# anovos/anovos

Measured on AMD Instinct MI355X. Metric: rows/sec (whole node) full analyzer+drift+transform, higher is better.
Workload: dtype fp32 data + fp64 accumulators; 1 GPU; model=anovos-full-pipeline, rows_per_gpu=125000000, n_cols=201, global_batch=125000000, parallelism=dp1

## Files before the change

anovos_amd/data_analyzer/quality_checker.py:

```python

from __future__ import annotations

import re
import warnings
from typing import Dict, List

import numpy as np
import pandas as pd
import torch

from anovos_amd.core import dist
from anovos_amd.core.dtypes import NULL_CODE
from anovos_amd.core.frame import AnovosFrame, Column
from anovos_amd.data_analyzer.stats_generator import (
    measures_of_cardinality,
    missingCount_computation,
    mode_computation,
    uniqueCount_computation,
)
from anovos_amd.data_transformer.transformers import _load_model, _save_model, imputation_MMM
from anovos_amd.ops import histogram as hist_ops
from anovos_amd.ops import rowops
from anovos_amd.ops import stats as stats_ops
from anovos_amd.shared.utils import attributeType_segregation, get_dtype, normalize_columns
# ... 51 lines not shown

@traced
def nullRows_detection(ctx, idf, list_of_cols="all", drop_cols=[], treatment=False, treatment_threshold=0.8, print_impact=False):
    if list_of_cols == "all":
        num_cols, cat_cols, _ = attributeType_segregation(idf)
        list_of_cols = num_cols + cat_cols
    cols = normalize_columns(idf, list_of_cols, drop_cols)
    if len(cols) == 0:
        raise TypeError("Invalid input for Column(s)")
    treatment = _parse_bool(treatment)
    treatment_threshold = float(treatment_threshold)
    if treatment_threshold < 0 or treatment_threshold > 1:
        raise TypeError("Invalid input for Treatment Threshold Value")

    counts = rowops.row_null_counts(idf, cols)
    if treatment_threshold == 1:
        flagged = counts == len(cols)
    else:
        flagged = counts > (len(cols) * treatment_threshold)

    total = idf.count()
    key = counts.to(torch.int32) * 2 + flagged.to(torch.int32)
    size = (len(cols) + 1) * 2
    from anovos_amd.ops import backend as _backend

    if key.is_cuda and _backend.use_hip(key):
        hist = _backend.hip_ext().code_counts(key.contiguous(), size).to(torch.float64)
    else:
        hist = torch.bincount(key.to(torch.long), minlength=size).to(torch.float64)
    dist.all_reduce_(hist, "sum")
    hist_l = hist.cpu().numpy().tolist()
    rows = []
    for nc in range(len(cols) + 1):
        for fl in (0, 1):
            c = hist_l[nc * 2 + fl]
            if c > 0:
                rows.append([nc, int(c), round(c / total, 4), fl])
    odf_print = pd.DataFrame(rows, columns=["null_cols_count", "row_count", "row_pct", "flagged"])

    if treatment:
        odf = idf.filter_rows(~flagged)
        odf_print = odf_print.rename(columns={"flagged": "treated"})
    else:
        odf = idf
    if print_impact:
        print(odf_print.to_string(index=False))
    return odf, odf_print


@traced
def nullColumns_detection(
    ctx,
    idf,
    list_of_cols="missing",
    drop_cols=[],
    treatment=False,
# ... 566 lines not shown
```

anovos_amd/ops/distinct.py:

```python

from __future__ import annotations

import math
from typing import Dict, List

import torch

from anovos_amd.core import dist
from anovos_amd.ops import backend
from anovos_amd.ops.groupby import _mix64

HLL_P = 12
HLL_M = 1 << HLL_P


def hll_registers(t: torch.Tensor, p: int = None) -> torch.Tensor:
    p = HLL_P if p is None else p
    m = 1 << p
    if t.is_cuda and backend.use_hip(t):
        ext = backend.hip_ext()
        return ext.hll_registers(t.contiguous(), p)
    v = t[~torch.isnan(t)]
    if v.dtype == torch.float32:
        x = v.view(torch.int32).to(torch.int64) & 0xFFFFFFFF
# ... 50 lines not shown
    zeros = int((regs == 0).sum())
    if e <= 2.5 * m and zeros:
        e = m * math.log(m / zeros)
    return e


def approx_distinct(idf, cols: List[str]) -> Dict[str, int]:
    out = {}
    if not cols:
        return out
    first = idf.col(cols[0]).data
    if first.is_cuda and backend.use_hip(first):
        ext = backend.hip_ext()
        cold = [c for c in cols if "moments" not in idf.col(c).cache]
        if len(cold) >= max(2, len(cols) // 2):
            from anovos_amd.ops import stats as stats_ops

            tensors = [idf.col(c).data.contiguous() for c in cols]
            shifts = stats_ops.compute_column_shifts(tensors)
            mom_local, flat = ext.moments_hll(tensors, HLL_P, shifts)
            glob = stats_ops.merge_moments_global(mom_local).numpy().tolist()
            for i, c in enumerate(cols):
                idf.col(c).cache.setdefault("moments", stats_ops.MomentStats(glob[i], shift=shifts[i]))
        else:
            flat = ext.hll_registers_multi([idf.col(c).data.contiguous() for c in cols], HLL_P)
    else:
        flat = torch.stack([hll_registers(idf.col(c).data) for c in cols]).to(torch.int32)
    dist.all_reduce_(flat, "max")
    regs = flat.cpu().numpy()
    import numpy as np

    m = float(HLL_M)
    z = np.power(2.0, -regs.astype(np.float64)).sum(axis=1)
    alpha = 0.7213 / (1 + 1.079 / m)
    e = alpha * m * m / z
# ... 31 lines not shown
```

anovos_amd/ops/groupby.py:

```python

from __future__ import annotations

from typing import Dict, List, Optional, Tuple

import torch

from anovos_amd.core import dist
from anovos_amd.core.dtypes import NULL_CODE
from anovos_amd.ops import backend


def align_dictionaries(idf, cols: List[str]) -> None:
    if not dist.is_dist():
        return
    cat = [
        c for c in cols
        if idf.col(c).kind == "categorical" and "dict_aligned" not in idf.col(c).cache
    ]
    if not cat:
        return
    import hashlib

    sigs = []
    for c in cat:
# ... 16 lines not shown
        col.cache.clear()
    for c in cat:
        idf.col(c).cache["dict_aligned"] = True


def cat_value_counts(idf, cols: List[str]) -> Dict[str, torch.Tensor]:
    align_dictionaries(idf, cols)
    out = {}
    cached = [c for c in cols if "cat_counts" in idf.col(c).cache]
    for c in cached:
        out[c] = idf.col(c).cache["cat_counts"]
    cols = [c for c in cols if c not in set(cached)]
    bufs = []
    gpu_cols = [c for c in cols if idf.col(c).data.is_cuda and backend.use_hip(idf.col(c).data)]
    if gpu_cols:
        ext = backend.hip_ext()
        sizes = [len(idf.col(c).dictionary or []) for c in gpu_cols]
        flat_multi = ext.code_counts_multi([idf.col(c).data.contiguous() for c in gpu_cols], sizes)
        gpu_cnt = {}
        off = 0
        for c, size in zip(gpu_cols, sizes):
            gpu_cnt[c] = flat_multi[off : off + size]
            gpu_cnt[c + "\0null"] = flat_multi[off + size : off + size + 1]
            off += size + 1
    for c in cols:
        col = idf.col(c)
        size = len(col.dictionary or [])
        codes = col.data
        if c in gpu_cols:
            cnt = gpu_cnt[c]
        else:
            valid = codes[codes != NULL_CODE].long()
            cnt = torch.bincount(valid, minlength=size) if size else torch.zeros(0, dtype=torch.int64, device=codes.device)
# ... 202 lines not shown
```

anovos_amd/ops/hip/anovos_bindings.hip:

```cpp

#include <torch/extension.h>
#include <c10/hip/HIPStream.h>
#include <hip/hip_runtime.h>

#include <algorithm>
#include <cstdlib>
#include <cstring>
#include <vector>

#include "anovos_kernels.h"

namespace {

hipStream_t current_stream() { return c10::hip::getCurrentHIPStream().stream(); }

void check_hip(int err, const char *what) {
  TORCH_CHECK(err == 0, what, " failed: ", hipGetErrorString((hipError_t)err));
}

int pick_chunks(int64_t n, int ncols) {
  int64_t by_size = (n + (1 << 16) - 1) >> 16;
  int64_t cap = std::max<int64_t>(1, 16384 / std::max(1, ncols));
  int64_t c = std::min<int64_t>(std::max<int64_t>(by_size, 1), cap);
  int64_t floor_c = std::min<int64_t>(by_size, std::max<int64_t>(1, 2048 / std::max(1, ncols)));
// ... 118 lines not shown
};

CutoffTable cutoff_table(const std::vector<torch::Tensor> &cutoffs, const std::vector<int64_t> &idx) {
  CutoffTable ct;
  for (int64_t i : idx) {
    auto cc = cutoffs[i].to(torch::kFloat64).cpu().contiguous();
    const double *cd = cc.data_ptr<double>();
    ct.offs.push_back((int64_t)ct.flat.size());
    ct.flat.insert(ct.flat.end(), cd, cd + cc.numel());
    ct.lens.push_back((int)cc.numel());
    ct.max_ncut = std::max(ct.max_ncut, (int)cc.numel());
  }
  return ct;
}

std::tuple<torch::Tensor, torch::Tensor> moments_body(const std::vector<torch::Tensor> &cols,
                                                      const std::vector<double> &shifts,
                                                      int64_t p, const char *name) {
  ColumnBatch all = gather_columns(cols, name, F32 | F64);
  if (!shifts.empty()) check_count(shifts.size(), cols.size(), name, "shifts");
  auto device = all.device;
  const bool hll = p >= 0;
  const int64_t m = hll ? (int64_t)1 << p : 0;
  auto mom = torch::zeros({all.ncols(), 9}, on(device, torch::kFloat64));
  torch::Tensor regs, reg_sub;
  if (hll) regs = torch::zeros({all.ncols(), m}, on(device, torch::kInt32));
  for (auto &b : split_by_dtype(all)) {
    int ncols = b.ncols();
    int nchunks = pick_chunks(b.maxn, ncols);
    auto dptr = upload(b.ptrs, device);
    auto dlen = upload(b.lens, device);
    auto dsh = upload(shifts.empty() ? std::vector<double>(ncols, 0.0) : pick(shifts, b.idx), device);
    auto partials = torch::empty({(int64_t)ncols * nchunks, 9}, on(device, torch::kFloat64));
    auto sub = torch::empty({ncols, 9}, on(device, torch::kFloat64));
    if (hll) {
      reg_sub = torch::zeros({ncols, m}, on(device, torch::kInt32));
      check_hip(anovos_moments_hll(ptr_table<const void>(dptr), dlen.data_ptr<int64_t>(),
                                   dsh.data_ptr<double>(), ncols, (int)p, nchunks, b.dtype,
                                   partials.data_ptr<double>(), sub.data_ptr<double>(),
                                   reg_sub.data_ptr<int>(), current_stream()),
                "anovos_moments_hll");
    } else {
      check_hip(anovos_moments(ptr_table<const void>(dptr), dlen.data_ptr<int64_t>(),
                               dsh.data_ptr<double>(), ncols, nchunks, b.dtype,
                               partials.data_ptr<double>(), sub.data_ptr<double>(),
                               current_stream()),
                "anovos_moments");
    }
    auto didx = upload(b.idx, device);
    mom.index_copy_(0, didx, sub);
    if (hll) regs.index_copy_(0, didx, reg_sub);
  }
  return {mom, regs};
}

// ... 68 lines not shown
  auto doff = upload(offs, b.device);
  auto dflat = upload(flat, b.device);
  check_hip(launch(ptr_table<const int32_t>(dptr), dlen.data_ptr<int64_t>(), b.ncols(),
                   dflat.template data_ptr<T>(), doff.data_ptr<int64_t>(), nchunks,
                   ptr_table<T>(dout), current_stream()),
            name);
  return outs;
}

}

torch::Tensor column_moments(std::vector<torch::Tensor> cols, std::vector<double> shifts) {
  return std::get<0>(moments_body(cols, shifts, -1, "column_moments"));
}

std::tuple<torch::Tensor, torch::Tensor> moments_hll(std::vector<torch::Tensor> cols, int64_t p,
                                                     std::vector<double> shifts) {
  TORCH_CHECK(p >= 0, "moments_hll: p must not be negative");
  return moments_body(cols, shifts, p, "moments_hll");
}

torch::Tensor column_histograms(std::vector<torch::Tensor> cols, torch::Tensor lo,
                                torch::Tensor hi, int64_t nbins) {
  ColumnBatch all = gather_columns(cols, "column_histograms", F32 | F64);
  auto device = all.device;
  auto lo_d = device_f64(lo, cols.size(), all, "lo");
  auto hi_d = device_f64(hi, cols.size(), all, "hi");
  auto out = torch::zeros({all.ncols(), nbins}, on(device, torch::kInt64));
  for (auto &b : split_by_dtype(all)) {
    int nchunks = pick_chunks(b.maxn, b.ncols());
    auto dptr = upload(b.ptrs, device);
    auto dlen = upload(b.lens, device);
    auto didx = upload(b.idx, device);
    auto sub = torch::zeros({b.ncols(), nbins}, on(device, torch::kInt64));
// ... 70 lines not shown
  check_hip(anovos_code_counts(codes.data_ptr<int32_t>(), codes.numel(), (int)size, nchunks,
                               (uint64_t *)out.data_ptr<int64_t>(), current_stream()),
            "anovos_code_counts");
  return out;
}

torch::Tensor hll_registers(torch::Tensor x, int64_t p) {
  ColumnBatch b = gather_columns({x}, "hll_registers", F32 | F64);
  auto regs = torch::zeros({(int64_t)1 << p}, on(b.device, torch::kInt32));
  if (x.numel() == 0) return regs;
  int nchunks = std::min(pick_chunks(x.numel(), 1), 4096);
  check_hip(anovos_hll(x.data_ptr(), x.numel(), (int)p, nchunks, b.dtype,
                       regs.data_ptr<int32_t>(), current_stream()),
            "anovos_hll");
  return regs;
}

void row_null_counts_num(std::vector<torch::Tensor> cols, torch::Tensor out) {
  ColumnBatch all = gather_columns(cols, "row_null_counts_num", F32 | F64 | I32, true);
  check_dense_on_device(out, all, "out", torch::kInt32, all.maxn);
  for (auto &b : split_by_dtype(all)) {
    auto dptr = upload(b.ptrs, b.device);
    check_hip(anovos_row_null(ptr_table<const void>(dptr), b.ncols(), out.numel(), b.dtype,
                              out.data_ptr<int32_t>(), current_stream()),
              "anovos_row_null");
  }
}

torch::Tensor hll_registers_multi(std::vector<torch::Tensor> cols, int64_t p) {
  ColumnBatch all = gather_columns(cols, "hll_registers_multi", F32 | F64);
// ... 168 lines not shown
              "anovos_centered_gram_sr");
    return gram;
  }
  int row_chunks = (int)std::min<int64_t>(std::max<int64_t>(1, 2048 / std::max(npairs, 1)),
                                          std::max<int64_t>(1, n >> 16));
  row_chunks = std::max(row_chunks, 1);
  auto partials = torch::empty({(int64_t)npairs * row_chunks, 256}, on(device, torch::kFloat32));
  check_hip(anovos_centered_gram(ptr_table<const void>(dptr), n, k, means_d.data_ptr<float>(),
                                 pi.data_ptr<int>(), pj.data_ptr<int>(), npairs, row_chunks,
                                 partials.data_ptr<float>(), gram.data_ptr<float>(),
                                 current_stream()),
            "anovos_centered_gram");
  return gram;
}

torch::Tensor code_counts_multi(std::vector<torch::Tensor> cols, std::vector<int64_t> sizes) {
  ColumnBatch b = gather_columns(cols, "code_counts_multi", I32);
  check_count(sizes.size(), cols.size(), b.name, "sizes");
  std::vector<int64_t> offs;
  int64_t off = 0;
  int lds_slots = 0;
  for (int64_t s : sizes) {
    TORCH_CHECK(s >= 0 && s < INT32_MAX, b.name, ": dictionary size out of range");
    offs.push_back(off);
    off += s + 1;
    if (s + 1 <= CODE_LDS_SLOTS) lds_slots = std::max(lds_slots, (int)s + 1);
  }
  int nchunks = pick_chunks(b.maxn, b.ncols());
  auto out = torch::zeros({off}, on(b.device, torch::kInt64));
  auto dptr = upload(b.ptrs, b.device);
  auto dlen = upload(b.lens, b.device);
  auto doff = upload(offs, b.device);
  auto dsz = upload(std::vector<int>(sizes.begin(), sizes.end()), b.device);
  check_hip(anovos_code_counts_multi(ptr_table<const int32_t>(dptr), dlen.data_ptr<int64_t>(),
                                     doff.data_ptr<int64_t>(), dsz.data_ptr<int>(), b.ncols(),
                                     lds_slots, nchunks, (uint64_t *)out.data_ptr<int64_t>(),
                                     current_stream()),
            "anovos_code_counts_multi");
  return out;
}

namespace {

struct PairPlan {
  std::vector<int64_t> items;
  std::vector<int64_t> offs;
  int64_t total = 0;
  int nitems = 0;
  int lds_slots = 0;
  int64_t col_reads = 0;
};

PairPlan plan_pair_items(const std::vector<int64_t> &sizes, const std::vector<int64_t> &pair_i,
                         const std::vector<int64_t> &pair_j) {
// ... 308 lines not shown
    auto sub = torch::zeros({b.ncols(), 2}, on(device, torch::kInt64));
    torch::Tensor dout;
    if (mode) dout = upload(out_ptrs(outs, b), device);
    check_hip(anovos_outlier_clamp(ptr_table<const void>(dptr), dlen.data_ptr<int64_t>(),
                                   b.ncols(), lo_sel.data_ptr<double>(), hi_sel.data_ptr<double>(),
                                   nchunks, (int)mode, b.dtype,
                                   mode ? ptr_table<void>(dout) : nullptr,
                                   (uint64_t *)sub.data_ptr<int64_t>(), current_stream()),
              "anovos_outlier_clamp");
    counts.index_copy_(0, didx, sub);
  }
  return {counts, outs};
}

PYBIND11_MODULE(TORCH_EXTENSION_NAME, m) {
  m.def("code_counts_multi", &code_counts_multi, "fused multi-column code counts + null slot (K5)");
  m.def("pair_code_counts", &pair_code_counts, "contingency tables of code-column pairs (K22)");
  m.def("pair_code_counts_plan", &pair_code_counts_plan,
        "[items, column streams, LDS counters] of a K22 pair list");
  m.def("grouped_moments", &grouped_moments, "(n, s1, s2) of value columns per code slot (K23)");
  m.def("grouped_moments_plan", &grouped_moments_plan,
        "[items, column streams, accumulator cells] of a K23 pair list");
  m.attr("GRP_CELLS") = GRP_CELLS;
  m.def("outlier_clamp_columns", &outlier_clamp_columns, "fused outlier count/clamp (K10/K11)");
  m.def("label_counts_multi", &label_counts_multi, "fused multi-column label-conditioned histograms (K9)");
  m.def("bucketize_label_counts", &bucketize_label_counts, "fused bucketize + label counts, no binned materialization (K6+K9)");
  m.def("moments_hll", &moments_hll, "fused moments + HLL registers (K1/K2+K4)",
        py::arg("cols"), py::arg("p"), py::arg("shifts") = std::vector<double>());
  m.def("centered_gram_bf16", &centered_gram_bf16, "bf16 MFMA centered Gram X^T X (K8)");
  m.def("bracket_histograms_grouped", &bracket_histograms_grouped, "grouped refinement histograms (K3)");
  m.def("bucketize_columns_float", &bucketize_columns_float, "bucketize to float bin labels (K6)");
  m.def("bucketize_columns_float_counts", &bucketize_columns_float_counts,
        "bucketize to float bin labels + per-column bin counts from the same pass (K6)");
  m.def("lut_apply_f32", &lut_apply_f32, "fused LUT gather -> float (K12)");
  m.def("lut_apply_i32", &lut_apply_i32, "fused LUT gather -> int32 (K12)");
  m.def("hll_registers_multi", &hll_registers_multi, "fused multi-column HLL (K4)");
  m.def("scale_columns", &scale_columns, "fused (x-a)*b scaling (K11)");
  m.def("fill_nan_columns", &fill_nan_columns, "fused NaN fill (K11)");
  m.def("fill_code_columns", &fill_code_columns, "fused categorical null fill (K11)");
  m.def("column_moments", &column_moments, "fused per-column moments (K1/K2)",
        py::arg("cols"), py::arg("shifts") = std::vector<double>());
  m.def("column_histograms", &column_histograms, "fused per-column histograms (K3/K6)");
  m.def("bracket_histograms", &bracket_histograms, "quantile-refinement histograms (K3)");
  m.def("bucketize_columns", &bucketize_columns, "branchless bucketize (K6)");
  m.def("code_counts", &code_counts, "dictionary code bincount (K5)");
  m.def("hll_registers", &hll_registers, "HyperLogLog registers (K4)");
  m.def("row_null_counts_num", &row_null_counts_num, "fused row null counts (K10)");
}
```

anovos_amd/ops/hip/anovos_kernels.h:

```cpp

#pragma once

#include <hip/hip_runtime.h>
#include <cstdint>


constexpr int CODE_LDS_SLOTS = 16384;
constexpr int PAIR_LDS_SLOTS = 16384;
constexpr int PAIR_PMAX = 8;
constexpr int PAIR_ITEM_WORDS = 4 + 4 * PAIR_PMAX;
constexpr int GRP_CELLS = 16;
constexpr int GRP_PMAX = 8;
constexpr int GRP_THREADS = 256;
constexpr int GRP_CELL_BYTES = 20;
constexpr int GRP_ITEM_WORDS = 5 + 2 * GRP_PMAX;
constexpr int RB_BINS = 512;
constexpr int RB_MAXB = 16;
constexpr int LABEL_MAX_SLOTS = 8192;
constexpr int BKT_COUNTS_MAX_NCUT = 4096;


extern "C" {
int anovos_moments(const void *const *cols, const int64_t *lens,
                   const double *shifts, int ncols, int nchunks, int dtype,
                   double *partials, double *out, hipStream_t stream);
int anovos_hist(const void *const *cols, const int64_t *lens, int ncols,
                const double *lo, const double *hi, int nbins, int nchunks,
                int dtype, uint64_t *out, hipStream_t stream);
int anovos_bracket_hist(const void *const *cols, const int64_t *lens,
                        const int64_t *colidx, int nbrackets, const double *lo,
                        const double *hi, int nbins, int nchunks, int dtype,
                        uint64_t *out, hipStream_t stream);
int anovos_bucketize(const void *const *cols, const int64_t *lens, int ncols,
                     const double *cutflat, const int64_t *cutoff_off,
// ... 28 lines not shown
                                  const int *cutoff_len, int max_ncut, int nchunks, int dtype,
                                  float *const *outs, uint64_t *counts, const int64_t *count_off,
                                  hipStream_t stream);
int anovos_lut_apply_f32(const int32_t *const *cols, const int64_t *lens, int ncols,
                         const float *lutflat, const int64_t *lut_off, int nchunks,
                         float *const *outs, hipStream_t stream);
int anovos_lut_apply_i32(const int32_t *const *cols, const int64_t *lens, int ncols,
                         const int32_t *lutflat, const int64_t *lut_off, int nchunks,
                         int32_t *const *outs, hipStream_t stream);
int anovos_fill_code(const int32_t *const *cols, const int64_t *lens, int ncols,
                     const int32_t *fill, int nchunks, int32_t *const *outs,
                     hipStream_t stream);
int anovos_code_counts_multi(const int32_t *const *cols, const int64_t *lens,
                             const int64_t *offs, const int *sizes, int ncols,
                             int lds_slots, int nchunks, uint64_t *out,
                             hipStream_t stream);
int anovos_outlier_clamp(const void *const *cols, const int64_t *lens,
                         int ncols, const double *lo, const double *hi,
                         int nchunks, int mode, int dtype, void *const *outs,
                         uint64_t *counts, hipStream_t stream);
int anovos_moments_hll(const void *const *cols, const int64_t *lens,
                       const double *shifts, int ncols, int p, int nchunks,
                       int dtype, double *partials, double *mom_out,
                       int32_t *regs, hipStream_t stream);
int anovos_bucketize_label_counts(const void *const *cols, const uint8_t *label,
                                  const int64_t *lens, const double *cutflat,
                                  const int64_t *cutoff_off, const int *cutoff_len,
                                  const int64_t *offs, const int *sizes, int ncols,
                                  int max_ncut, int max_slots, int nchunks,
                                  int dtype, uint64_t *out, hipStream_t stream);
int anovos_label_counts_multi(const void *const *cols, const uint8_t *label,
                              const int64_t *lens, const int64_t *offs,
                              const int *sizes, const int *dtypes, int ncols,
                              int max_slots, int nchunks, uint64_t *out,
                              hipStream_t stream);
int anovos_centered_gram(const void *const *cols, int64_t n, int k,
                         const float *means, const int *pair_i,
                         const int *pair_j, int npairs, int row_chunks,
                         float *partials, float *gram, hipStream_t stream);
// ... 14 lines not shown
```

anovos_amd/ops/hip/anovos_kernels.hip:

```cpp

#include <hip/hip_runtime.h>
#include <cfloat>
#include <cstdint>
#include <cmath>

#include "anovos_kernels.h"

#define THREADS 256
#define DEV_INLINE __device__ __forceinline__

typedef int nat_i4 __attribute__((ext_vector_type(4)));
typedef float nat_f4 __attribute__((ext_vector_type(4)));


#define NSTAT 9

struct MomAcc {
  double n, s1, s2, s3, s4, mn, mx, zn, nf;
};

DEV_INLINE void mom_add(MomAcc &a, double v, double shift) {
  if (!isnan(v)) {
    a.n += 1.0;
    double d = v - shift;
    a.s1 += d;
    double d2 = d * d;
    a.s2 += d2;
// ... 750 lines not shown
  __syncthreads();
  for (int c = c0; c < c1; ++c) {
    const T *__restrict__ x = cols[c] + s;
    for (int i = threadIdx.x; i < nr; i += THREADS)
      if (is_null_elem(x[i])) rc[i] += 1;
  }
  __syncthreads();
  if (ncolchunks == 1) {
    for (int i = threadIdx.x; i < nr; i += THREADS) out[s + i] += (int32_t)rc[i];
  } else {
    for (int i = threadIdx.x; i < nr; i += THREADS)
      if (rc[i]) atomicAdd(&out[s + i], (int32_t)rc[i]);
  }
}


template <typename T>
__global__ __launch_bounds__(THREADS) void hll_multi_kernel(
    const T *const *cols, const int64_t *lens, int p, int nchunks,
    int32_t *regs ) {
  extern __shared__ int32_t sreg[];
  const int m = 1 << p;
  const int col = blockIdx.x / nchunks;
  const int chunk = blockIdx.x % nchunks;
  for (int i = threadIdx.x; i < m; i += THREADS) sreg[i] = 0;
  __syncthreads();
  const T *__restrict__ x = cols[col];
  const int64_t n = lens[col];
  const int64_t per = (n + nchunks - 1) / nchunks;
  const int64_t s = (int64_t)chunk * per;
// ... 342 lines not shown
                   void *const *outs, hipStream_t stream) {
  dim3 grid(ncols * nchunks);
  if (dtype == 0)
    hipLaunchKernelGGL(fillnan_kernel<float>, grid, dim3(THREADS), 0, stream,
                       (const float *const *)cols, lens, fill, nchunks,
                       (float *const *)outs);
  else
    hipLaunchKernelGGL(fillnan_kernel<double>, grid, dim3(THREADS), 0, stream,
                       (const double *const *)cols, lens, fill, nchunks,
                       (double *const *)outs);
  return (int)hipGetLastError();
}

}

__global__ __launch_bounds__(THREADS) void code_counts_multi_kernel(
    const int32_t *const *cols, const int64_t *lens, const int64_t *offs,
    const int *sizes, int nchunks, uint64_t *out) {
  const int col = blockIdx.x / nchunks;
  const int chunk = blockIdx.x % nchunks;
  const int32_t *__restrict__ codes = cols[col];
  const int64_t n = lens[col];
  const int size = sizes[col];
  const int slots = size + 1;
  uint64_t *base = out + offs[col];

  extern __shared__ uint32_t cnt[];
  const bool use_lds = (slots <= CODE_LDS_SLOTS);
  if (use_lds) {
    for (int i = threadIdx.x; i < slots; i += THREADS) cnt[i] = 0;
    __syncthreads();
  }
  const int64_t per = (n + nchunks - 1) / nchunks;
  const int64_t s = (int64_t)chunk * per;
  const int64_t e = min(n, s + per);
  if (use_lds) {
    const int64_t nv = (e - s) / 4;
    const nat_i4 *__restrict__ cv = reinterpret_cast<const nat_i4 *>(codes + s);
    for (int64_t i = threadIdx.x; i < nv; i += THREADS) {
      nat_i4 c = __builtin_nontemporal_load(&cv[i]);
      atomicAdd(&cnt[(c.x >= 0 && c.x < size) ? c.x : size], 1u);
      atomicAdd(&cnt[(c.y >= 0 && c.y < size) ? c.y : size], 1u);
      atomicAdd(&cnt[(c.z >= 0 && c.z < size) ? c.z : size], 1u);
      atomicAdd(&cnt[(c.w >= 0 && c.w < size) ? c.w : size], 1u);
    }
    for (int64_t i = s + nv * 4 + threadIdx.x; i < e; i += THREADS) {
      int c = codes[i];
      atomicAdd(&cnt[(c >= 0 && c < size) ? c : size], 1u);
    }
    __syncthreads();
    for (int i = threadIdx.x; i < slots; i += THREADS)
      if (cnt[i]) atomicAdd((unsigned long long *)&base[i], (unsigned long long)cnt[i]);
  } else {
    for (int64_t i = s + threadIdx.x; i < e; i += THREADS) {
      int c = codes[i];
      atomicAdd((unsigned long long *)&base[(c >= 0 && c < size) ? c : size], 1ull);
    }
  }
}

template <typename T>
__global__ __launch_bounds__(THREADS) void outlier_clamp_kernel(
// ... 85 lines not shown
      red[1][threadIdx.x] += red[1][threadIdx.x + st];
    }
    __syncthreads();
  }
  if (threadIdx.x == 0) {
    if (red[0][0]) atomicAdd((unsigned long long *)&counts[col * 2 + 0], (unsigned long long)red[0][0]);
    if (red[1][0]) atomicAdd((unsigned long long *)&counts[col * 2 + 1], (unsigned long long)red[1][0]);
  }
}

extern "C" {

int anovos_code_counts_multi(const int32_t *const *cols, const int64_t *lens,
                             const int64_t *offs, const int *sizes, int ncols,
                             int lds_slots, int nchunks, uint64_t *out,
                             hipStream_t stream) {
  if (lds_slots < 0 || lds_slots > CODE_LDS_SLOTS) return (int)hipErrorInvalidValue;
  size_t lds = (size_t)lds_slots * 4;
  hipLaunchKernelGGL(code_counts_multi_kernel, dim3(ncols * nchunks),
                     dim3(THREADS), lds, stream, cols, lens, offs, sizes,
                     nchunks, out);
  return (int)hipGetLastError();
}

int anovos_outlier_clamp(const void *const *cols, const int64_t *lens,
                         int ncols, const double *lo, const double *hi,
                         int nchunks, int mode, int dtype, void *const *outs,
                         uint64_t *counts, hipStream_t stream) {
  if (dtype == 0)
    hipLaunchKernelGGL(outlier_clamp_kernel<float>, dim3(ncols * nchunks),
                       dim3(THREADS), 0, stream, (const float *const *)cols,
                       lens, lo, hi, nchunks, mode, (float *const *)outs,
                       counts);
  else
    hipLaunchKernelGGL(outlier_clamp_kernel<double>, dim3(ncols * nchunks),
                       dim3(THREADS), 0, stream, (const double *const *)cols,
                       lens, lo, hi, nchunks, mode, (double *const *)outs,
                       counts);
  return (int)hipGetLastError();
}

}

template <typename T>
__global__ __launch_bounds__(THREADS) void moments_hll_kernel(
    const T *const *cols, const int64_t *lens, const double *shifts, int p,
    int nchunks, double *partials, int32_t *regs ) {
  extern __shared__ int32_t sreg[];
  const int m = 1 << p;
  const int col = blockIdx.x / nchunks;
  const int chunk = blockIdx.x % nchunks;
  for (int i = threadIdx.x; i < m; i += THREADS) sreg[i] = 0;
  __syncthreads();

  const T *__restrict__ x = cols[col];
  const int64_t n = lens[col];
  const double shift = shifts ? shifts[col] : 0.0;
  const int64_t per = (n + nchunks - 1) / nchunks;
  const int64_t s = (int64_t)chunk * per;
  const int64_t e = min(n, s + per);

  MomAcc a{0, 0, 0, 0, 0, (double)INFINITY, -(double)INFINITY, 0};
  auto body = [&](T v) {
    mom_add(a, (double)v, shift);
    int idx, rho;
    if (hll_hash(v, p, idx, rho)) { if (sreg[idx] < rho) atomicMax(&sreg[idx], rho); }
  };
  if (sizeof(T) == 4) {
    const int64_t nv = (e - s) / 4;
    const float4 *xv = reinterpret_cast<const float4 *>(x + s);
    for (int64_t i = threadIdx.x; i < nv; i += THREADS) {
      float4 v = xv[i];
      body((T)v.x);
      body((T)v.y);
      body((T)v.z);
      body((T)v.w);
    }
    for (int64_t i = s + nv * 4 + threadIdx.x; i < e; i += THREADS) body(x[i]);
  } else {
    for (int64_t i = s + threadIdx.x; i < e; i += THREADS) body(x[i]);
  }

  mom_block_reduce_write(a, &partials[(int64_t)blockIdx.x * NSTAT]);
  int32_t *g = &regs[(int64_t)col * m];
  for (int i = threadIdx.x; i < m; i += THREADS)
    if (sreg[i]) atomicMax(&g[i], sreg[i]);
}

extern "C" int anovos_moments_hll(const void *const *cols, const int64_t *lens,
                                  const double *shifts, int ncols, int p,
                                  int nchunks, int dtype, double *partials,
                                  double *mom_out, int32_t *regs,
                                  hipStream_t stream) {
  dim3 grid(ncols * nchunks);
  size_t lds = (size_t)(1 << p) * 4;
  if (dtype == 0)
    hipLaunchKernelGGL(moments_hll_kernel<float>, grid, dim3(THREADS), lds, stream,
                       (const float *const *)cols, lens, shifts, p, nchunks, partials, regs);
  else
    hipLaunchKernelGGL(moments_hll_kernel<double>, grid, dim3(THREADS), lds, stream,
                       (const double *const *)cols, lens, shifts, p, nchunks, partials, regs);
  hipLaunchKernelGGL(moments_reduce_kernel, dim3(ncols), dim3(THREADS), 0, stream,
                     partials, nchunks, mom_out);
  return (int)hipGetLastError();
}

DEV_INLINE int label_slot_f32(float v, int slots) {
  if (v != v) return 0;
  const int slot = (int)fminf(fmaxf(v, -1.0f), (float)(slots - 1)) + 1;
  return (slot >= slots) ? slots - 1 : slot;
}

__global__ __launch_bounds__(THREADS) void label_counts_multi_kernel(
    const void *const *cols, const uint8_t *__restrict__ label,
    const int64_t *lens, const int64_t *offs, const int *sizes,
    const int *dtypes, int nchunks, uint64_t *out) {
// ... 264 lines not shown
```

anovos_amd/ops/rowops.py:

```python

from __future__ import annotations

from typing import List

import torch

from anovos_amd.ops import backend


def row_null_counts(idf, cols: List[str]) -> torch.Tensor:
    n = idf.local_rows()
    dev = idf.device
    first = idf.col(cols[0]).data if cols else None
    if first is not None and first.is_cuda and backend.use_hip(first):
        ext = backend.hip_ext()
        fused = [idf.col(c).data.contiguous() for c in cols
                 if idf.col(c).kind == "numerical" or idf.col(c).data.dtype == torch.int32]
        rest = [c for c in cols
                if not (idf.col(c).kind == "numerical" or idf.col(c).data.dtype == torch.int32)]
        out = torch.zeros(n, dtype=torch.int32, device=dev)
        if fused:
            ext.row_null_counts_num(fused, out)
        for c in rest:
            out += idf.col(c).null_mask().to(torch.int32)
        return out
    out = torch.zeros(n, dtype=torch.int32, device=dev)
    for c in cols:
        out += idf.col(c).null_mask().to(torch.int32)
    return out
```

Baseline: 431.8 million rows/sec.

## Emit per-column null bitmasks during moments/HLL and code-count passes for row null counts

The fused moments+HLL and code-count kernels now also write wave-ballot null bitmasks per column, and these are stored in the column cache. row_null_counts then reads the bitmasks (one bit per row) instead of rescanning the full fp32/int32 columns. nullRows_detection also histograms the raw null counts and derives the flag per bucket on the host, which drops the key tensor and the flagged-tensor build. In exchange, the earlier passes do extra ballots and mask stores and hold extra device memory, and the cached masks must stay valid for the frame.

```diff
diff --git a/anovos_amd/data_analyzer/quality_checker.py b/anovos_amd/data_analyzer/quality_checker.py
--- a/anovos_amd/data_analyzer/quality_checker.py
+++ b/anovos_amd/data_analyzer/quality_checker.py
@@ -89,32 +89,32 @@
         raise TypeError("Invalid input for Treatment Threshold Value")
 
     counts = rowops.row_null_counts(idf, cols)
-    if treatment_threshold == 1:
-        flagged = counts == len(cols)
-    else:
-        flagged = counts > (len(cols) * treatment_threshold)
+
+    def flag(t):
+        if treatment_threshold == 1:
+            return t == len(cols)
+        return t > (len(cols) * treatment_threshold)
 
     total = idf.count()
-    key = counts.to(torch.int32) * 2 + flagged.to(torch.int32)
-    size = (len(cols) + 1) * 2
+    size = len(cols) + 1
     from anovos_amd.ops import backend as _backend
 
-    if key.is_cuda and _backend.use_hip(key):
-        hist = _backend.hip_ext().code_counts(key.contiguous(), size).to(torch.float64)
-    else:
-        hist = torch.bincount(key.to(torch.long), minlength=size).to(torch.float64)
+    if counts.is_cuda and _backend.use_hip(counts):
+        hist = _backend.hip_ext().code_counts(counts.contiguous(), size).to(torch.float64)
+    else:
+        hist = torch.bincount(counts.to(torch.long), minlength=size).to(torch.float64)
     dist.all_reduce_(hist, "sum")
     hist_l = hist.cpu().numpy().tolist()
+    bucket_flag = flag(torch.arange(size, dtype=torch.int32)).tolist()
     rows = []
-    for nc in range(len(cols) + 1):
-        for fl in (0, 1):
-            c = hist_l[nc * 2 + fl]
-            if c > 0:
-                rows.append([nc, int(c), round(c / total, 4), fl])
+    for nc in range(size):
+        c = hist_l[nc]
+        if c > 0:
+            rows.append([nc, int(c), round(c / total, 4), int(bucket_flag[nc])])
     odf_print = pd.DataFrame(rows, columns=["null_cols_count", "row_count", "row_pct", "flagged"])
 
     if treatment:
-        odf = idf.filter_rows(~flagged)
+        odf = idf.filter_rows(~flag(counts))
         odf_print = odf_print.rename(columns={"flagged": "treated"})
     else:
         odf = idf
diff --git a/anovos_amd/ops/distinct.py b/anovos_amd/ops/distinct.py
--- a/anovos_amd/ops/distinct.py
+++ b/anovos_amd/ops/distinct.py
@@ -88,11 +88,16 @@
         ext = backend.hip_ext()
         cold = [c for c in cols if "moments" not in idf.col(c).cache]
         if len(cold) >= max(2, len(cols) // 2):
+            from anovos_amd.ops import rowops
             from anovos_amd.ops import stats as stats_ops
 
             tensors = [idf.col(c).data.contiguous() for c in cols]
             shifts = stats_ops.compute_column_shifts(tensors)
-            mom_local, flat = ext.moments_hll(tensors, HLL_P, shifts)
+            if rowops.null_masks_enabled():
+                mom_local, flat, masks, parts = ext.moments_hll(tensors, HLL_P, shifts, null_masks=True)
+                rowops.store_null_masks(idf, cols, masks, parts)
+            else:
+                mom_local, flat = ext.moments_hll(tensors, HLL_P, shifts)
             glob = stats_ops.merge_moments_global(mom_local).numpy().tolist()
             for i, c in enumerate(cols):
                 idf.col(c).cache.setdefault("moments", stats_ops.MomentStats(glob[i], shift=shifts[i]))
diff --git a/anovos_amd/ops/groupby.py b/anovos_amd/ops/groupby.py
--- a/anovos_amd/ops/groupby.py
+++ b/anovos_amd/ops/groupby.py
@@ -54,9 +54,16 @@
     bufs = []
     gpu_cols = [c for c in cols if idf.col(c).data.is_cuda and backend.use_hip(idf.col(c).data)]
     if gpu_cols:
+        from anovos_amd.ops import rowops
+
         ext = backend.hip_ext()
         sizes = [len(idf.col(c).dictionary or []) for c in gpu_cols]
-        flat_multi = ext.code_counts_multi([idf.col(c).data.contiguous() for c in gpu_cols], sizes)
+        codes_multi = [idf.col(c).data.contiguous() for c in gpu_cols]
+        if rowops.null_masks_enabled():
+            flat_multi, masks, parts = ext.code_counts_multi(codes_multi, sizes, null_masks=True)
+            rowops.store_null_masks(idf, gpu_cols, masks, parts)
+        else:
+            flat_multi = ext.code_counts_multi(codes_multi, sizes)
         gpu_cnt = {}
         off = 0
         for c, size in zip(gpu_cols, sizes):
diff --git a/anovos_amd/ops/hip/anovos_bindings.hip b/anovos_amd/ops/hip/anovos_bindings.hip
--- a/anovos_amd/ops/hip/anovos_bindings.hip
+++ b/anovos_amd/ops/hip/anovos_bindings.hip
@@ -156,9 +156,23 @@
   return ct;
 }
 
+struct NullMasks {
+  std::vector<torch::Tensor> masks;
+  std::vector<std::vector<int64_t>> parts;
+  explicit NullMasks(size_t ncols) : masks(ncols), parts(ncols) {}
+
+  int64_t add(int64_t i, int64_t n, int nchunks, const torch::Device &dev) {
+    const int64_t per = (n + nchunks - 1) / nchunks;
+    masks[i] = torch::empty({nchunks * null_mask_chunk_words(per)}, on(dev, torch::kInt64));
+    parts[i] = {n, (int64_t)nchunks, per};
+    return (int64_t)masks[i].data_ptr();
+  }
+};
+
 std::tuple<torch::Tensor, torch::Tensor> moments_body(const std::vector<torch::Tensor> &cols,
                                                       const std::vector<double> &shifts,
-                                                      int64_t p, const char *name) {
+                                                      int64_t p, const char *name,
+                                                      NullMasks *nm = nullptr) {
   ColumnBatch all = gather_columns(cols, name, F32 | F64);
   if (!shifts.empty()) check_count(shifts.size(), cols.size(), name, "shifts");
   auto device = all.device;
@@ -177,10 +191,18 @@
     auto sub = torch::empty({ncols, 9}, on(device, torch::kFloat64));
     if (hll) {
       reg_sub = torch::zeros({ncols, m}, on(device, torch::kInt32));
+      torch::Tensor dmask;
+      if (nm && b.dtype == 0) {
+        std::vector<int64_t> mptrs;
+        for (int j = 0; j < ncols; ++j) mptrs.push_back(nm->add(b.idx[j], b.lens[j], nchunks, device));
+        dmask = upload(mptrs, device);
+      }
       check_hip(anovos_moments_hll(ptr_table<const void>(dptr), dlen.data_ptr<int64_t>(),
                                    dsh.data_ptr<double>(), ncols, (int)p, nchunks, b.dtype,
                                    partials.data_ptr<double>(), sub.data_ptr<double>(),
-                                   reg_sub.data_ptr<int>(), current_stream()),
+                                   reg_sub.data_ptr<int>(),
+                                   dmask.defined() ? ptr_table<uint64_t>(dmask) : nullptr,
+                                   current_stream()),
                 "anovos_moments_hll");
     } else {
       check_hip(anovos_moments(ptr_table<const void>(dptr), dlen.data_ptr<int64_t>(),
@@ -279,10 +301,13 @@
   return std::get<0>(moments_body(cols, shifts, -1, "column_moments"));
 }
 
-std::tuple<torch::Tensor, torch::Tensor> moments_hll(std::vector<torch::Tensor> cols, int64_t p,
-                                                     std::vector<double> shifts) {
+py::object moments_hll(std::vector<torch::Tensor> cols, int64_t p, std::vector<double> shifts,
+                       bool null_masks) {
   TORCH_CHECK(p >= 0, "moments_hll: p must not be negative");
-  return moments_body(cols, shifts, p, "moments_hll");
+  if (!null_masks) return py::cast(moments_body(cols, shifts, p, "moments_hll"));
+  NullMasks nm(cols.size());
+  auto r = moments_body(cols, shifts, p, "moments_hll", &nm);
+  return py::make_tuple(std::get<0>(r), std::get<1>(r), nm.masks, nm.parts);
 }
 
 torch::Tensor column_histograms(std::vector<torch::Tensor> cols, torch::Tensor lo,
@@ -383,6 +408,35 @@
                        regs.data_ptr<int32_t>(), current_stream()),
             "anovos_hll");
   return regs;
+}
+
+void row_null_counts_masked(std::vector<torch::Tensor> masks, std::vector<int64_t> partition,
+                            torch::Tensor out) {
+  const char *name = "row_null_counts_masked";
+  TORCH_CHECK(!masks.empty(), name, ": no columns");
+  check_count(partition.size(), 3, name, "partition");
+  const int64_t n = partition[0], nchunks = partition[1], per = partition[2];
+  TORCH_CHECK(n >= 0 && nchunks >= 1 && nchunks <= INT32_MAX && per == (n + nchunks - 1) / nchunks,
+              name, ": partition is not {n, nchunks, ceil(n / nchunks)}");
+  auto device = masks[0].device();
+  TORCH_CHECK(device.is_cuda(), name, ": device masks required");
+  const int64_t words = nchunks * null_mask_chunk_words(per);
+  std::vector<int64_t> ptrs;
+  for (auto &t : masks) {
+    TORCH_CHECK(t.device() == device && t.is_contiguous() && t.scalar_type() == torch::kInt64, name,
+                ": masks must be contiguous int64 tensors on one device");
+    TORCH_CHECK(t.numel() == words, name, ": a mask has ", t.numel(), " words, its partition needs ",
+                words);
+    TORCH_CHECK((int64_t)t.data_ptr() % 32 == 0, name, ": masks must be 32-byte aligned");
+    ptrs.push_back((int64_t)t.data_ptr());
+  }
+  TORCH_CHECK(out.device() == device && out.is_contiguous() && out.scalar_type() == torch::kInt32,
+              name, ": out must be a contiguous int32 tensor on the masks' device");
+  TORCH_CHECK(out.numel() == n, name, ": mask/out length mismatch");
+  auto dptr = upload(ptrs, device);
+  check_hip(anovos_row_null_masked(ptr_table<const uint64_t>(dptr), (int)ptrs.size(), n,
+                                   (int)nchunks, per, out.data_ptr<int32_t>(), current_stream()),
+            "anovos_row_null_masked");
 }
 
 void row_null_counts_num(std::vector<torch::Tensor> cols, torch::Tensor out) {
@@ -581,7 +635,8 @@
   return gram;
 }
 
-torch::Tensor code_counts_multi(std::vector<torch::Tensor> cols, std::vector<int64_t> sizes) {
+py::object code_counts_multi(std::vector<torch::Tensor> cols, std::vector<int64_t> sizes,
+                             bool null_masks) {
   ColumnBatch b = gather_columns(cols, "code_counts_multi", I32);
   check_count(sizes.size(), cols.size(), b.name, "sizes");
   std::vector<int64_t> offs;
@@ -599,12 +654,22 @@
   auto dlen = upload(b.lens, b.device);
   auto doff = upload(offs, b.device);
   auto dsz = upload(std::vector<int>(sizes.begin(), sizes.end()), b.device);
+  NullMasks nm(cols.size());
+  torch::Tensor dmask;
+  if (null_masks) {
+    std::vector<int64_t> mptrs;
+    for (int j = 0; j < b.ncols(); ++j)
+      mptrs.push_back(sizes[j] + 1 <= CODE_LDS_SLOTS ? nm.add(j, b.lens[j], nchunks, b.device) : 0);
+    dmask = upload(mptrs, b.device);
+  }
   check_hip(anovos_code_counts_multi(ptr_table<const int32_t>(dptr), dlen.data_ptr<int64_t>(),
                                      doff.data_ptr<int64_t>(), dsz.data_ptr<int>(), b.ncols(),
                                      lds_slots, nchunks, (uint64_t *)out.data_ptr<int64_t>(),
+                                     null_masks ? ptr_table<uint64_t>(dmask) : nullptr,
                                      current_stream()),
             "anovos_code_counts_multi");
-  return out;
+  if (!null_masks) return py::cast(out);
+  return py::make_tuple(out, nm.masks, nm.parts);
 }
 
 namespace {
@@ -943,7 +1008,8 @@
 }
 
 PYBIND11_MODULE(TORCH_EXTENSION_NAME, m) {
-  m.def("code_counts_multi", &code_counts_multi, "fused multi-column code counts + null slot (K5)");
+  m.def("code_counts_multi", &code_counts_multi, "fused multi-column code counts + null slot (K5)",
+        py::arg("cols"), py::arg("sizes"), py::arg("null_masks") = false);
   m.def("pair_code_counts", &pair_code_counts, "contingency tables of code-column pairs (K22)");
   m.def("pair_code_counts_plan", &pair_code_counts_plan,
         "[items, column streams, LDS counters] of a K22 pair list");
@@ -955,7 +1021,8 @@
   m.def("label_counts_multi", &label_counts_multi, "fused multi-column label-conditioned histograms (K9)");
   m.def("bucketize_label_counts", &bucketize_label_counts, "fused bucketize + label counts, no binned materialization (K6+K9)");
   m.def("moments_hll", &moments_hll, "fused moments + HLL registers (K1/K2+K4)",
-        py::arg("cols"), py::arg("p"), py::arg("shifts") = std::vector<double>());
+        py::arg("cols"), py::arg("p"), py::arg("shifts") = std::vector<double>(),
+        py::arg("null_masks") = false);
   m.def("centered_gram_bf16", &centered_gram_bf16, "bf16 MFMA centered Gram X^T X (K8)");
   m.def("bracket_histograms_grouped", &bracket_histograms_grouped, "grouped refinement histograms (K3)");
   m.def("bucketize_columns_float", &bucketize_columns_float, "bucketize to float bin labels (K6)");
@@ -975,4 +1042,6 @@
   m.def("code_counts", &code_counts, "dictionary code bincount (K5)");
   m.def("hll_registers", &hll_registers, "HyperLogLog registers (K4)");
   m.def("row_null_counts_num", &row_null_counts_num, "fused row null counts (K10)");
-}
+  m.def("row_null_counts_masked", &row_null_counts_masked,
+        "row null counts from null lane masks (K10m)");
+}
diff --git a/anovos_amd/ops/hip/anovos_kernels.h b/anovos_amd/ops/hip/anovos_kernels.h
--- a/anovos_amd/ops/hip/anovos_kernels.h
+++ b/anovos_amd/ops/hip/anovos_kernels.h
@@ -18,6 +18,9 @@
 constexpr int RB_MAXB = 16;
 constexpr int LABEL_MAX_SLOTS = 8192;
 constexpr int BKT_COUNTS_MAX_NCUT = 4096;
+__host__ __device__ constexpr int64_t null_mask_chunk_words(int64_t per) {
+  return 4 * ((((per >> 2) + 63) >> 6) + 1);
+}
 
 
 extern "C" {
@@ -76,7 +79,7 @@
 int anovos_code_counts_multi(const int32_t *const *cols, const int64_t *lens,
                              const int64_t *offs, const int *sizes, int ncols,
                              int lds_slots, int nchunks, uint64_t *out,
-                             hipStream_t stream);
+                             uint64_t *const *masks, hipStream_t stream);
 int anovos_outlier_clamp(const void *const *cols, const int64_t *lens,
                          int ncols, const double *lo, const double *hi,
                          int nchunks, int mode, int dtype, void *const *outs,
@@ -84,7 +87,10 @@
 int anovos_moments_hll(const void *const *cols, const int64_t *lens,
                        const double *shifts, int ncols, int p, int nchunks,
                        int dtype, double *partials, double *mom_out,
-                       int32_t *regs, hipStream_t stream);
+                       int32_t *regs, uint64_t *const *masks, hipStream_t stream);
+int anovos_row_null_masked(const uint64_t *const *masks, int ncols, int64_t n,
+                           int nchunks, int64_t per, int32_t *out,
+                           hipStream_t stream);
 int anovos_bucketize_label_counts(const void *const *cols, const uint8_t *label,
                                   const int64_t *lens, const double *cutflat,
                                   const int64_t *cutoff_off, const int *cutoff_len,
diff --git a/anovos_amd/ops/hip/anovos_kernels.hip b/anovos_amd/ops/hip/anovos_kernels.hip
--- a/anovos_amd/ops/hip/anovos_kernels.hip
+++ b/anovos_amd/ops/hip/anovos_kernels.hip
@@ -11,6 +11,35 @@
 
 typedef int nat_i4 __attribute__((ext_vector_type(4)));
 typedef float nat_f4 __attribute__((ext_vector_type(4)));
+
+DEV_INLINE uint64_t *null_masks_first_group(uint64_t *chunk_words) {
+  return chunk_words + 4 * __builtin_amdgcn_readfirstlane((int)(threadIdx.x >> 6));
+}
+
+DEV_INLINE void null_masks_store(uint64_t *group, uint64_t b0, uint64_t b1, uint64_t b2,
+                                 uint64_t b3) {
+  if ((threadIdx.x & 63) == 0) {
+    typedef uint64_t nat_u2 __attribute__((ext_vector_type(2)));
+    nat_u2 *g = reinterpret_cast<nat_u2 *>(group);
+    g[0] = nat_u2{b0, b1};
+    g[1] = nat_u2{b2, b3};
+  }
+}
+
+DEV_INLINE void null_masks_emit(uint64_t *group, bool n0, bool n1, bool n2, bool n3) {
+  null_masks_store(group, __ballot(n0), __ballot(n1), __ballot(n2), __ballot(n3));
+}
+
+DEV_INLINE void null_masks_emit_valid(uint64_t *group, bool v0, bool v1, bool v2, bool v3) {
+  const uint64_t act = __ballot(true);
+  null_masks_store(group, act & ~__ballot(v0), act & ~__ballot(v1), act & ~__ballot(v2),
+                   act & ~__ballot(v3));
+}
+
+DEV_INLINE void null_masks_emit_tail(uint64_t *group, bool isnull) {
+  const uint64_t b = __ballot(isnull);
+  if (threadIdx.x == 0) group[0] = b;
+}
 
 
 #define NSTAT 9
@@ -791,6 +820,78 @@
   }
 }
 
+typedef uint64_t nat_u64x4 __attribute__((ext_vector_type(4)));
+#define NULL_MASK_UNROLL 8
+
+DEV_INLINE nat_u64x4 load_mask_group(const uint64_t *group) {
+  typedef const nat_u64x4 __attribute__((address_space(4))) *const_group;
+  return *(const_group)(uintptr_t)group;
+}
+
+__global__ __launch_bounds__(THREADS) void row_null_masked_kernel(
+    const uint64_t *const *__restrict__ masks, int ncols, int64_t n, int nchunks, int64_t per,
+    int32_t *__restrict__ out) {
+  const int64_t wpc = null_mask_chunk_words(per);
+  const int64_t gpc = wpc >> 2;
+  const int lane = threadIdx.x & 63;
+  const int wave = __builtin_amdgcn_readfirstlane((int)(threadIdx.x >> 6));
+  const int64_t item = (int64_t)blockIdx.x * (THREADS / 64) + wave;
+  if (item >= gpc * nchunks) return;
+  const int64_t chunk = item / gpc;
+  const int64_t G = item % gpc;
+  const int64_t s = chunk * per;
+  const int64_t e = min(n, s + per);
+  if (e <= s) return;
+  const int64_t nv = (e - s) >> 2;
+  const int64_t gv = (nv + 63) >> 6;
+  const int ntail = (int)((e - s) - 4 * nv);
+  const bool tail = (G == gv);
+  if (G > gv || (tail && ntail == 0)) return;
+
+  const int64_t woff = chunk * wpc + 4 * G;
+  uint32_t c0 = 0, c1 = 0, c2 = 0, c3 = 0;
+  auto add = [&](nat_u64x4 w) {
+    c0 += __builtin_amdgcn_inverse_ballot_w64(w.x);
+    c1 += __builtin_amdgcn_inverse_ballot_w64(w.y);
+    c2 += __builtin_amdgcn_inverse_ballot_w64(w.z);
+    c3 += __builtin_amdgcn_inverse_ballot_w64(w.w);
+  };
+  int c = 0;
+  for (; c + NULL_MASK_UNROLL <= ncols; c += NULL_MASK_UNROLL) {
+    nat_u64x4 w[NULL_MASK_UNROLL];
+#pragma unroll
+    for (int j = 0; j < NULL_MASK_UNROLL; ++j) w[j] = load_mask_group(masks[c + j] + woff);
+#pragma unroll
+    for (int j = 0; j < NULL_MASK_UNROLL; ++j) add(w[j]);
+  }
+  for (; c < ncols; ++c) add(load_mask_group(masks[c] + woff));
+  if (tail) {
+    if (lane < ntail) out[s + 4 * nv + lane] += (int32_t)c0;
+    return;
+  }
+  const int64_t q = 64 * G + lane;
+  if (q < nv) {
+    int32_t *o = out + s + 4 * q;
+    o[0] += (int32_t)c0;
+    o[1] += (int32_t)c1;
+    o[2] += (int32_t)c2;
+    o[3] += (int32_t)c3;
+  }
+}
+
+extern "C" int anovos_row_null_masked(const uint64_t *const *masks, int ncols, int64_t n,
+                                      int nchunks, int64_t per, int32_t *out,
+                                      hipStream_t stream) {
+  if (n <= 0 || ncols <= 0) return 0;
+  if (nchunks < 1 || per != (n + nchunks - 1) / nchunks) return (int)hipErrorInvalidValue;
+  const int64_t items = (null_mask_chunk_words(per) >> 2) * nchunks;
+  const int64_t blocks = (items + THREADS / 64 - 1) / (THREADS / 64);
+  if (blocks > INT32_MAX) return (int)hipErrorInvalidValue;
+  hipLaunchKernelGGL(row_null_masked_kernel, dim3((uint32_t)blocks), dim3(THREADS), 0, stream,
+                     masks, ncols, n, nchunks, per, out);
+  return (int)hipGetLastError();
+}
+
 
 template <typename T>
 __global__ __launch_bounds__(THREADS) void hll_multi_kernel(
@@ -1163,9 +1264,10 @@
 
 }
 
+template <bool MASK>
 __global__ __launch_bounds__(THREADS) void code_counts_multi_kernel(
     const int32_t *const *cols, const int64_t *lens, const int64_t *offs,
-    const int *sizes, int nchunks, uint64_t *out) {
+    const int *sizes, int nchunks, uint64_t *out, uint64_t *const *masks) {
   const int col = blockIdx.x / nchunks;
   const int chunk = blockIdx.x % nchunks;
   const int32_t *__restrict__ codes = cols[col];
@@ -1186,8 +1288,17 @@
   if (use_lds) {
     const int64_t nv = (e - s) / 4;
     const nat_i4 *__restrict__ cv = reinterpret_cast<const nat_i4 *>(codes + s);
+    uint64_t *mrow = nullptr, *mgroup = nullptr;
+    if (MASK) {
+      mrow = masks[col] + (int64_t)chunk * null_mask_chunk_words(per);
+      mgroup = null_masks_first_group(mrow);
+    }
     for (int64_t i = threadIdx.x; i < nv; i += THREADS) {
       nat_i4 c = __builtin_nontemporal_load(&cv[i]);
+      if (MASK) {
+        null_masks_emit(mgroup, c.x == -1, c.y == -1, c.z == -1, c.w == -1);
+        mgroup += 4 * (THREADS / 64);
+      }
       atomicAdd(&cnt[(c.x >= 0 && c.x < size) ? c.x : size], 1u);
       atomicAdd(&cnt[(c.y >= 0 && c.y < size) ? c.y : size], 1u);
       atomicAdd(&cnt[(c.z >= 0 && c.z < size) ? c.z : size], 1u);
@@ -1195,6 +1306,7 @@
     }
     for (int64_t i = s + nv * 4 + threadIdx.x; i < e; i += THREADS) {
       int c = codes[i];
+      if (MASK) null_masks_emit_tail(mrow + 4 * ((nv + 63) >> 6), c == -1);
       atomicAdd(&cnt[(c >= 0 && c < size) ? c : size], 1u);
     }
     __syncthreads();
@@ -1310,12 +1422,17 @@
 int anovos_code_counts_multi(const int32_t *const *cols, const int64_t *lens,
                              const int64_t *offs, const int *sizes, int ncols,
                              int lds_slots, int nchunks, uint64_t *out,
-                             hipStream_t stream) {
+                             uint64_t *const *masks, hipStream_t stream) {
   if (lds_slots < 0 || lds_slots > CODE_LDS_SLOTS) return (int)hipErrorInvalidValue;
   size_t lds = (size_t)lds_slots * 4;
-  hipLaunchKernelGGL(code_counts_multi_kernel, dim3(ncols * nchunks),
-                     dim3(THREADS), lds, stream, cols, lens, offs, sizes,
-                     nchunks, out);
+  if (masks)
+    hipLaunchKernelGGL(code_counts_multi_kernel<true>, dim3(ncols * nchunks),
+                       dim3(THREADS), lds, stream, cols, lens, offs, sizes,
+                       nchunks, out, masks);
+  else
+    hipLaunchKernelGGL(code_counts_multi_kernel<false>, dim3(ncols * nchunks),
+                       dim3(THREADS), lds, stream, cols, lens, offs, sizes,
+                       nchunks, out, masks);
   return (int)hipGetLastError();
 }
 
@@ -1338,10 +1455,11 @@
 
 }
 
-template <typename T>
+template <typename T, bool MASK>
 __global__ __launch_bounds__(THREADS) void moments_hll_kernel(
     const T *const *cols, const int64_t *lens, const double *shifts, int p,
-    int nchunks, double *partials, int32_t *regs ) {
+    int nchunks, double *partials, int32_t *regs ,
+    uint64_t *const *masks) {
   extern __shared__ int32_t sreg[];
   const int m = 1 << p;
   const int col = blockIdx.x / nchunks;
@@ -1365,14 +1483,26 @@
   if (sizeof(T) == 4) {
     const int64_t nv = (e - s) / 4;
     const float4 *xv = reinterpret_cast<const float4 *>(x + s);
+    uint64_t *mrow = nullptr, *mgroup = nullptr;
+    if (MASK) {
+      mrow = masks[col] + (int64_t)chunk * null_mask_chunk_words(per);
+      mgroup = null_masks_first_group(mrow);
+    }
     for (int64_t i = threadIdx.x; i < nv; i += THREADS) {
       float4 v = xv[i];
+      if (MASK) {
+        null_masks_emit_valid(mgroup, !isnan(v.x), !isnan(v.y), !isnan(v.z), !isnan(v.w));
+        mgroup += 4 * (THREADS / 64);
+      }
       body((T)v.x);
       body((T)v.y);
       body((T)v.z);
       body((T)v.w);
     }
-    for (int64_t i = s + nv * 4 + threadIdx.x; i < e; i += THREADS) body(x[i]);
+    for (int64_t i = s + nv * 4 + threadIdx.x; i < e; i += THREADS) {
+      if (MASK) null_masks_emit_tail(mrow + 4 * ((nv + 63) >> 6), isnan((float)x[i]));
+      body(x[i]);
+    }
   } else {
     for (int64_t i = s + threadIdx.x; i < e; i += THREADS) body(x[i]);
   }
@@ -1387,15 +1517,22 @@
                                   const double *shifts, int ncols, int p,
                                   int nchunks, int dtype, double *partials,
                                   double *mom_out, int32_t *regs,
-                                  hipStream_t stream) {
+                                  uint64_t *const *masks, hipStream_t stream) {
   dim3 grid(ncols * nchunks);
   size_t lds = (size_t)(1 << p) * 4;
-  if (dtype == 0)
-    hipLaunchKernelGGL(moments_hll_kernel<float>, grid, dim3(THREADS), lds, stream,
-                       (const float *const *)cols, lens, shifts, p, nchunks, partials, regs);
+  if (masks && dtype != 0) return (int)hipErrorInvalidValue;
+  if (masks)
+    hipLaunchKernelGGL((moments_hll_kernel<float, true>), grid, dim3(THREADS), lds, stream,
+                       (const float *const *)cols, lens, shifts, p, nchunks, partials, regs,
+                       masks);
+  else if (dtype == 0)
+    hipLaunchKernelGGL((moments_hll_kernel<float, false>), grid, dim3(THREADS), lds, stream,
+                       (const float *const *)cols, lens, shifts, p, nchunks, partials, regs,
+                       masks);
   else
-    hipLaunchKernelGGL(moments_hll_kernel<double>, grid, dim3(THREADS), lds, stream,
-                       (const double *const *)cols, lens, shifts, p, nchunks, partials, regs);
+    hipLaunchKernelGGL((moments_hll_kernel<double, false>), grid, dim3(THREADS), lds, stream,
+                       (const double *const *)cols, lens, shifts, p, nchunks, partials, regs,
+                       masks);
   hipLaunchKernelGGL(moments_reduce_kernel, dim3(ncols), dim3(THREADS), 0, stream,
                      partials, nchunks, mom_out);
   return (int)hipGetLastError();
diff --git a/anovos_amd/ops/rowops.py b/anovos_amd/ops/rowops.py
--- a/anovos_amd/ops/rowops.py
+++ b/anovos_amd/ops/rowops.py
@@ -1,11 +1,24 @@
 
 from __future__ import annotations
 
+import os
 from typing import List
 
 import torch
 
 from anovos_amd.ops import backend
+
+NULL_MASK_KEY = "null_mask"
+
+
+def null_masks_enabled() -> bool:
+    return os.environ.get("ANOVOS_NULL_MASKS", "1") != "0"
+
+
+def store_null_masks(idf, cols: List[str], masks, parts) -> None:
+    for c, m, p in zip(cols, masks, parts):
+        if m is not None:
+            idf.col(c).cache[NULL_MASK_KEY] = (m, tuple(int(v) for v in p))
 
 
 def row_null_counts(idf, cols: List[str]) -> torch.Tensor:
@@ -14,11 +27,21 @@
     first = idf.col(cols[0]).data if cols else None
     if first is not None and first.is_cuda and backend.use_hip(first):
         ext = backend.hip_ext()
-        fused = [idf.col(c).data.contiguous() for c in cols
+        groups = {}
+        scan = []
+        for c in cols:
+            hit = idf.col(c).cache.get(NULL_MASK_KEY)
+            if hit is not None and hit[1][0] == n and hit[0].device == first.device:
+                groups.setdefault(hit[1], []).append(hit[0])
+            else:
+                scan.append(c)
+        fused = [idf.col(c).data.contiguous() for c in scan
                  if idf.col(c).kind == "numerical" or idf.col(c).data.dtype == torch.int32]
-        rest = [c for c in cols
+        rest = [c for c in scan
                 if not (idf.col(c).kind == "numerical" or idf.col(c).data.dtype == torch.int32)]
         out = torch.zeros(n, dtype=torch.int32, device=dev)
+        for part, masks in groups.items():
+            ext.row_null_counts_masked(masks, list(part), out)
         if fused:
             ext.row_null_counts_num(fused, out)
         for c in rest:
```

Result: faster. 451.8 million rows/sec, median of 6 (+4.6%).
